# s-esposito/MonoGS

Measured on AMD Instinct MI355X. Metric: rasteriser fwd+bwd Mpix/s @1080p, higher is better.
Workload: dtype f32; 1 GPU; C5: 2000000 Gaussians, 1920x1080, fwd+bwd, seeded synthetic map (SURVEY.md 8d), one keyframe per GPU; gaussians=2000000, width=1920, height=1080, settle_steps=60, instance_count=device-side (capacity mode, overflow checked), parallelism=keyframe-per-gpu x1

## Files before the change

### include/monogs_raster.h

```cpp
#ifndef MONOGS_RASTER_H
#define MONOGS_RASTER_H

#include <stddef.h>
#include <stdint.h>

#ifdef __cplusplus
extern "C" {
#endif

#define MGS_ABI_VERSION 19
#define MGS_TILE 16

typedef struct mgs_camera {
    int32_t image_height;
    int32_t image_width;
    float tanfovx;
    float tanfovy;
    float scale_modifier;
    int32_t sh_degree;
    int32_t sh_coeffs;
    int32_t scale_dim;
    int32_t flags;
    const float* bg;
    const float* viewmatrix;
    const float* projmatrix;
    const float* projmatrix_raw;
    const float* campos;
} mgs_camera;

#define MGS_FLAG_EXCLUSIVE_DEVICE 1

typedef struct mgs_timing {
    float preprocess_ms;
// ... 25 lines not shown
                           const float* opacities,
                           const float* scales,
                           const float* rotations,
                           const float* cov3D_precomp,
                           void* geometry, int32_t* radii ,
                           void* prepare_backward ,
                           uint64_t* num_rendered ,
                           const uint32_t* prev_status ,
                           uint32_t* prev_status_out ,
                           mgs_timing* timing , void* stream);

int mgs_forward_render(const mgs_camera* cam, int32_t P, uint64_t num_rendered,
                       void* geometry, void* binning, void* image,
                       float* out_color, float* out_depth, float* out_opacity, int32_t* n_touched,
                       uint32_t* status ,
                       mgs_timing* timing, void* stream);

#define MGS_STATUS_CAPACITY_OVERFLOW 1u
#define MGS_STATUS_DEPTH_SORT_TIMEOUT 2u
#define MGS_STATUS_TILE_SORT_TIMEOUT 4u

int mgs_debug_set_radix_spin_limit(uint32_t limit);
int mgs_debug_set_option(const char* name, int64_t value);

int mgs_binning_path(int32_t P, int32_t W, int32_t H);

size_t mgs_debug_sort_temp_bytes(uint64_t n, int32_t bits);
int mgs_debug_sort_pairs(uint32_t* keys, uint32_t* vals, uint32_t* keys_alt, uint32_t* vals_alt, uint64_t n, int32_t bits,
                         void* temp, void* stream);

int mgs_forward_render_capacity(const mgs_camera* cam, int32_t P, uint64_t capacity,
                                void* geometry, void* binning, void* image,
                                float* out_color, float* out_depth, float* out_opacity, int32_t* n_touched,
                                uint32_t* overflow, mgs_timing* timing, void* stream);
int mgs_forward_capacity(const mgs_camera* cam, int32_t P, const float* means3D, const float* shs,
                         const float* colors_precomp, const float* opacities, const float* scales, const float* rotations,
                         const float* cov3D_precomp, void* geometry, int32_t* radii, void* prepare_backward,
                         uint64_t capacity, void* binning, void* image, float* out_color, float* out_depth,
                         float* out_opacity, int32_t* n_touched, uint32_t* overflow, mgs_timing* timing, void* stream);

int mgs_backward(const mgs_camera* cam, int32_t P, uint64_t num_rendered,
                 const float* means3D, const float* shs, const float* colors_precomp,
                 const float* opacities, const float* scales, const float* rotations,
                 const float* cov3D_precomp, const int32_t* radii,
                 const void* geometry, const void* binning, const void* image,
                 const float* dL_dcolor, const float* dL_ddepth,
// ... 221 lines not shown
```

### monogs_amd/_lib.py

```python
from __future__ import annotations

import ctypes as C
import os

_HERE = os.path.dirname(os.path.abspath(__file__))
LIB_PATH = os.environ.get("MGS_LIB_PATH") or os.path.join(_HERE, "lib", "libmonogs_raster.so")
ABI_VERSION = 19

c_float_p = C.c_void_p


class MgsCamera(C.Structure):
    _fields_ = [
        ("image_height", C.c_int32), ("image_width", C.c_int32),
        ("tanfovx", C.c_float), ("tanfovy", C.c_float), ("scale_modifier", C.c_float),
        ("sh_degree", C.c_int32), ("sh_coeffs", C.c_int32), ("scale_dim", C.c_int32), ("flags", C.c_int32),
        ("bg", C.c_void_p), ("viewmatrix", C.c_void_p), ("projmatrix", C.c_void_p),
        ("projmatrix_raw", C.c_void_p), ("campos", C.c_void_p),
    ]


class MgsTiming(C.Structure):
    _fields_ = [(n, C.c_float) for n in (
        "preprocess_ms", "depth_sort_ms", "scan_ms", "duplicate_ms", "sort_ms", "ranges_ms", "blend_fwd_ms",
        "blend_bwd_ms", "geom_bwd_ms")]

    def as_dict(self):
        return {n: float(getattr(self, n)) for n, _ in self._fields_}


# ... 33 lines not shown
    "mgs_forward_preprocess": (C.c_int, [C.POINTER(MgsCamera), C.c_int32] + [C.c_void_p] * 7
                               + [C.c_void_p, C.c_void_p, C.c_void_p, C.POINTER(C.c_uint64), C.c_void_p, C.POINTER(C.c_uint32),
                                  C.POINTER(MgsTiming), C.c_void_p]),
    "mgs_forward_capacity": (C.c_int, [C.POINTER(MgsCamera), C.c_int32] + [C.c_void_p] * 7 + [C.c_void_p] * 3 + [C.c_uint64]
                             + [C.c_void_p] * 7 + [C.POINTER(MgsTiming), C.c_void_p]),
    "mgs_forward_render": (C.c_int, [C.POINTER(MgsCamera), C.c_int32, C.c_uint64] + [C.c_void_p] * 8
                           + [C.POINTER(MgsTiming), C.c_void_p]),
    "mgs_debug_set_radix_spin_limit": (C.c_int, [C.c_uint32]),
    "mgs_debug_set_option": (C.c_int, [C.c_char_p, C.c_int64]),
    "mgs_binning_path": (C.c_int, [C.c_int32, C.c_int32, C.c_int32]),
    "mgs_debug_sort_temp_bytes": (C.c_size_t, [C.c_uint64, C.c_int32]),
    "mgs_debug_sort_pairs": (C.c_int, [C.c_void_p] * 4 + [C.c_uint64, C.c_int32, C.c_void_p, C.c_void_p]),
    "mgs_forward_render_capacity": (C.c_int, [C.POINTER(MgsCamera), C.c_int32, C.c_uint64] + [C.c_void_p] * 8
                                    + [C.POINTER(MgsTiming), C.c_void_p]),
    "mgs_backward": (C.c_int, [C.POINTER(MgsCamera), C.c_int32, C.c_uint64] + [C.c_void_p] * 7
                     + [C.c_void_p] * 4 + [C.c_void_p] * 4 + [C.c_void_p] * 9
                     + [C.c_void_p, C.c_int32, C.POINTER(MgsTiming), C.c_void_p]),
    "mgs_backward_tau": (C.c_void_p, [C.c_void_p, C.c_int32]),
    "mgs_debug_blend_stats": (C.c_int, [C.POINTER(MgsCamera), C.c_int32, C.c_uint64] + [C.c_void_p] * 5),
    "mgs_debug_blend_mask_stats": (C.c_int, [C.POINTER(MgsCamera), C.c_int32, C.c_uint64] + [C.c_void_p] * 5),
    "mgs_features_forward": (C.c_int, [C.POINTER(MgsCamera), C.c_int32, C.c_int32, C.c_uint64] + [C.c_void_p] * 7
                             + [C.c_float, C.c_void_p]),
    "mgs_features_backward": (C.c_int, [C.POINTER(MgsCamera), C.c_int32, C.c_int32, C.c_uint64] + [C.c_void_p] * 5 + [C.c_void_p]),
    "mgs_debug_valu_ceiling": (C.c_int, [C.c_void_p, C.c_int32, C.c_void_p]),
    "mgs_debug_set_blend_events": (C.c_int, [C.c_void_p] * 4),
    "mgs_debug_last_backward_split": (C.c_int, []),
    "mgs_mark_visible": (C.c_int, [C.c_int32, C.c_void_p, C.c_void_p, C.c_void_p, C.c_void_p, C.c_void_p]),
    "mgs_loss_scratch_bytes": (C.c_size_t, []),
    "mgs_loss_forward": (C.c_int, [C.c_int32] * 4 + [C.c_float] + [C.c_void_p] * 9 + [C.c_void_p, C.c_void_p, C.c_void_p]),
    "mgs_loss_backward": (C.c_int, [C.c_int32] * 4 + [C.c_float] + [C.c_void_p] * 9
                          + [C.c_void_p, C.c_void_p, C.c_void_p, C.c_void_p, C.c_void_p, C.c_void_p]),
    "mgs_loss_grads": (C.c_int, [C.c_int32] * 4 + [C.c_float] + [C.c_void_p] * 9 + [C.c_void_p] * 4),
    "mgs_ssim_scratch_bytes": (C.c_size_t, [C.c_int32] * 4),
    "mgs_ssim_forward": (C.c_int, [C.c_int32] * 5 + [C.c_float] * 2 + [C.c_void_p] * 5),
    "mgs_ssim_backward": (C.c_int, [C.c_int32] * 4 + [C.c_float] * 2 + [C.c_void_p] * 6),
    "mgs_refine_loss_forward": (C.c_int, [C.c_int32] * 2 + [C.c_float] + [C.c_void_p] * 5),
    "mgs_refine_loss_backward": (C.c_int, [C.c_int32] * 2 + [C.c_float] + [C.c_void_p] * 6),
    "mgs_refine_loss_grads": (C.c_int, [C.c_int32] * 2 + [C.c_float] + [C.c_void_p] * 5),
    "mgs_backproject": (C.c_int, [C.c_int32] * 3 + [C.c_void_p] * 6 + [C.c_float] * 4 + [C.c_void_p] * 6),
    "mgs_camera_setup": (C.c_int, [C.c_void_p] * 7),
    "mgs_pose_step": (C.c_int, [C.c_void_p] * 12 + [C.c_int32] + [C.c_float] * 7
                      + [C.c_void_p, C.c_void_p, C.c_int32, C.c_void_p] + [C.c_void_p] * 4 + [C.c_void_p]),
    "mgs_pose_step_batch": (C.c_int, [C.c_int32, C.POINTER(C.c_void_p)] + [C.c_float] * 7 + [C.c_int32, C.c_void_p]),
    "mgs_adam_step": (C.c_int, [C.c_int32] + [C.c_void_p] * 6 + [C.c_double] * 3 + [C.c_int32, C.c_void_p, C.c_void_p, C.c_void_p]),
    "mgs_window_stats": (C.c_int, [C.c_int32, C.c_int32] + [C.c_void_p] * 6 + [C.c_int32, C.c_void_p, C.c_void_p]),
    "mgs_window_apply": (C.c_int, [C.c_int32] + [C.c_void_p] * 7),
# ... 59 lines not shown
```

### monogs_amd/csrc/api.hip

```cpp
#include "common.h"

#include <stdarg.h>
#include <stdio.h>
#include <string.h>

namespace mgs {

static thread_local char g_err[512] = "";

void set_error(const char* fmt, ...) {
    va_list ap;
    va_start(ap, fmt);
    vsnprintf(g_err, sizeof(g_err), fmt, ap);
    va_end(ap);
}

static inline char* take(char*& p, size_t bytes) {
    char* r = p;
    p += align_up(bytes, 256);
    return r;
}

GeometryState GeometryState::carve(void* base, int P) {
    char* p = (char*)align_up((size_t)base, 256);
// ... 375 lines not shown
    MGS_HIP(zero_fill(stats_dev, MGS_BLEND_STATS_WORDS * sizeof(uint64_t), s));
    if (P == 0 || R == 0) return 0;
    const int W = cam->image_width, H = cam->image_height;
    GeometryState g = GeometryState::carve(const_cast<void*>(geometry), P);
    ImageState img = ImageState::carve(const_cast<void*>(image), W, H);
    BinningState b = BinningState::carve(const_cast<void*>(binning), R, W, H);
    return launch_blend_backward_stats(*cam, g, b, img, (unsigned long long*)stats_dev, s);
}

int mgs_debug_blend_mask_stats(const mgs_camera* cam, int32_t P, uint64_t R, const void* geometry, const void* binning,
                               const void* image, uint64_t* stats_dev, void* stream) {
    if (check_cam(cam)) return 1;
    if (!geometry || !image || !stats_dev || (R > 0 && !binning)) { set_error("bad arguments"); return 1; }
    hipStream_t s = (hipStream_t)stream;
    MGS_HIP(zero_fill(stats_dev, MGS_BLEND_MASK_STATS_WORDS * sizeof(uint64_t), s));
    if (P == 0 || R == 0) return 0;
    const int W = cam->image_width, H = cam->image_height;
    GeometryState g = GeometryState::carve(const_cast<void*>(geometry), P);
    ImageState img = ImageState::carve(const_cast<void*>(image), W, H);
    BinningState b = BinningState::carve(const_cast<void*>(binning), R, W, H);
    return launch_blend_mask_stats(*cam, g, b, img, (unsigned long long*)stats_dev, s);
}

int mgs_debug_valu_ceiling(float* out, int32_t iters, void* stream) {
    if (!out || iters < 1) { set_error("mgs_debug_valu_ceiling: bad arguments"); return 1; }
    return launch_valu_ceiling(out, iters, (hipStream_t)stream);
}

int mgs_debug_last_backward_split(void) { return g_dbg_last_bwd_split; }

int mgs_debug_set_radix_spin_limit(uint32_t limit) { return set_radix_spin_limit(limit); }

int mgs_debug_set_blend_events(void* fwd_start, void* fwd_end, void* bwd_start, void* bwd_end) {
    if ((fwd_start == nullptr) != (fwd_end == nullptr) || (bwd_start == nullptr) != (bwd_end == nullptr)) {
        set_error("mgs_debug_set_blend_events: a pair is both events or neither");
        return 1;
    }
    g_dbg_fwd_events[0] = (hipEvent_t)fwd_start; g_dbg_fwd_events[1] = (hipEvent_t)fwd_end;
    g_dbg_bwd_events[0] = (hipEvent_t)bwd_start; g_dbg_bwd_events[1] = (hipEvent_t)bwd_end;
    return 0;
}

static int g_opt_debug_sort_exclusive = 0;
size_t mgs_debug_sort_temp_bytes(uint64_t n, int32_t bits) { return radix_temp_bytes(n, bits); }
int mgs_debug_sort_pairs(uint32_t* keys, uint32_t* vals, uint32_t* keys_alt, uint32_t* vals_alt, uint64_t n, int32_t bits,
                         void* temp, void* stream) {
// ... 13 lines not shown
    uint32_t err[RADIX_ERROR_WORDS];
    MGS_HIP(hipMemcpyAsync(err, radix_error_flag(temp, n, bits), sizeof(err), hipMemcpyDeviceToHost, s));
    MGS_HIP(hipStreamSynchronize(s));
    if (err[0] | err[1] | err[2] | err[3]) { set_error("mgs_debug_sort_pairs: a look-back spin timed out"); return 2; }
    return 0;
}

int mgs_debug_set_option(const char* name, int64_t value) {
    if (name && !strcmp(name, "radix_scanned")) { g_opt_radix_scanned = (int)value; return 0; }
    if (name && !strcmp(name, "radix_ballot_rank")) { g_opt_radix_ballot_rank = (int)value; return 0; }
    if (name && !strcmp(name, "radix_xcd_band")) { g_opt_radix_xcd_band = (int)value; return 0; }
    if (name && !strcmp(name, "debug_sort_exclusive")) { g_opt_debug_sort_exclusive = (int)value; return 0; }
    if (name && !strcmp(name, "dup_slot_major")) { g_opt_dup_slot_major = (int)value; return 0; }
    if (name && !strcmp(name, "blend_bwd_transposed")) {
        g_opt_blend_bwd_transposed = value < 0 ? 2 : (int)value;
        g_opt_blend_bwd_transposed_set = value >= 0;
        return 0;
    }
    if (name && !strcmp(name, "blend_bwd_split")) { g_opt_blend_bwd_split = value < 0 ? -1 : (int)value; return 0; }
    if (name && !strcmp(name, "blend_bwd_split_min")) { g_opt_blend_bwd_split_min = value < 0 ? 4 : (int)value; return 0; }
    if (name && !strcmp(name, "blend_bwd_split_frac")) { g_opt_blend_bwd_split_frac = value < 0 ? 32 : (int)value; return 0; }
    if (name && !strcmp(name, "scan_small")) { g_opt_scan_small = (int)value; return 0; }
    if (name && !strcmp(name, "tile_sort_fused")) { g_opt_tile_sort_fused = value < 0 ? 1 : (int)value; return 0; }
    if (name && !strcmp(name, "knn_grid_min")) { g_opt_knn_grid_min = value > 0x7FFFFFFF ? 0x7FFFFFFF : (int)value; return 0; }
    set_error("mgs_debug_set_option: unknown option");
    return 1;
}

int mgs_mark_visible(int32_t P, const float* means3D, const float* viewmatrix, const float* projmatrix,
                     uint8_t* visible, void* stream) {
    (void)projmatrix;
    if (P < 0 || (P > 0 && (!means3D || !viewmatrix || !visible))) { set_error("bad arguments"); return 1; }
    return launch_mark_visible(P, means3D, viewmatrix, visible, (hipStream_t)stream);
}

size_t mgs_knn_scratch_bytes(int32_t P) { return knn_scratch_bytes(P); }

int mgs_dist2_knn(int32_t P, const float* points, float* out, void* scratch, void* stream) {
    if (P < 0 || (P > 0 && (!points || !out))) { set_error("bad arguments"); return 1; }
    return launch_knn(P, points, out, scratch, (hipStream_t)stream);
}

}
```

### monogs_amd/csrc/binning.hip

```cpp
#include "common.h"
#include "tile_sort.h"


namespace mgs {

constexpr int SCAN_THREADS = 256;
__device__ __forceinline__ int scan_nblocks_dev(int P) { return (P + SCAN_ITEMS - 1) / SCAN_ITEMS; }
constexpr int SCAN_PER_THREAD = SCAN_ITEMS / SCAN_THREADS;

__device__ __forceinline__ uint32_t wave_incl_scan(uint32_t v, int) { return wave_incl_scan_dpp(v); }

__device__ __forceinline__ uint32_t block_excl_scan(uint32_t v, uint32_t& total, uint32_t* smem ) {
    const int lane = threadIdx.x & 63, wv = threadIdx.x >> 6;
    const uint32_t incl = wave_incl_scan(v, lane);
    if (lane == 63) smem[wv] = incl;
    __syncthreads();
    uint32_t base = 0;
    for (int w = 0; w < wv; ++w) base += smem[w];
    total = smem[0] + smem[1] + smem[2] + smem[3];
    __syncthreads();
    return base + incl - v;
}

__device__ __forceinline__ uint32_t scan_block_rows(const uint2* __restrict__ rects, int n, int cbase, int lane, int wv,
// ... 104 lines not shown
    if (scan_is_small(P)) {
        hipLaunchKernelGGL(scan_small_kernel, dim3(nb), dim3(SCAN_THREADS), 0, s, rects, g.point_offsets, g.scan_blocks,
                           g.scan_status, P, nb, const_cast<uint32_t*>(radix_depth_error_flag(g.sort_temp, (uint64_t)P)),
                           exclusive ? 0 : 1);
        MGS_HIP(hipGetLastError());
        return 0;
    }
    hipLaunchKernelGGL(scan_local_kernel, dim3(nb), dim3(SCAN_THREADS), 0, s, rects, g.point_offsets,
                       g.scan_blocks, P);
    hipLaunchKernelGGL(scan_blocks_kernel, dim3(1), dim3(SCAN_THREADS), 0, s, g.scan_blocks, nb);
    MGS_HIP(hipGetLastError());
    return 0;
}

__device__ __forceinline__ void dup_pair(uint32_t gidx, const uint32_t* __restrict__ depth_key, int lo, uint32_t& val,
                                         uint32_t& kfield) {
    val = gidx; kfield = 0u;
    if (depth_key) {
        const uint32_t k = depth_key[gidx];
        const uint32_t d = k == 0xFFFFFFFFu ? DEPTH_KEY_NARROW : min(k - DEPTH_KEY_SUB, DEPTH_KEY_NARROW);
        kfield = d >> lo;
        if (lo) val |= (d & ((1u << lo) - 1u)) << (32 - lo);
    }
}
__global__ void __launch_bounds__(256) duplicate_kernel(int P, const uint2* __restrict__ rects,
                                                        const uint32_t* __restrict__ perm,
                                                        const uint32_t* __restrict__ depth_key, int tshift, int lo,
                                                        const uint32_t* __restrict__ offsets ,
                                                        const uint32_t* __restrict__ block_sums ,
                                                        uint32_t* keys,
                                                        uint32_t* vals, int gx, int gy, uint32_t r_cap,
                                                        int32_t* __restrict__ n_touched, uint2* __restrict__ ranges,
                                                        int ntiles, uint32_t* __restrict__ zero_ptr, size_t zero_words,
                                                        uint32_t* __restrict__ count, uint32_t* __restrict__ overflow,
                                                        const uint32_t* __restrict__ depth_err, int offsets_global,
                                                        uint32_t* __restrict__ hist , int hist_passes,
                                                        int n_threads , int slot_major,
                                                        unsigned long long* __restrict__ prepare ) {
    const int i = blockIdx.x * 256 + threadIdx.x;
    if (i == 0 && prepare) {
        prepare[1] = prepare[0];
        prepare[0] = 0ull;
    }
    const int lane = threadIdx.x & 63;
    grid_zero(zero_ptr, zero_words, (size_t)n_threads, 256);
    const bool depth_bad = depth_err && radix_failed(depth_err) != 0u;
    if (i == 0 && count) {
        const uint32_t R = (P > 0 && !depth_bad) ? block_sums[scan_nblocks_dev(P)] : 0u;
        count[0] = min(R, r_cap);
        count[1] = R > r_cap ? 1u : 0u;
    }
    if (i == 0 && overflow)
        overflow[0] = (count ? count[1] : 0u) | (depth_bad ? (uint32_t)MGS_STATUS_DEPTH_SORT_TIMEOUT : 0u);
    if (i < ntiles) ranges[i] = make_uint2(0xFFFFFFFFu, 0u);
    if (i < P) n_touched[i] = 0;
    uint32_t idx = 0, nt = 0, off = 0, kf = 0;
    int x0 = 0, y0 = 0, x1 = 0;
    if (i < P) {
        dup_pair(perm ? perm[i] : (uint32_t)i, depth_key, lo, idx, kf);
        const uint2 r = rects[i];
        const int w = (int)(r.y & 0xFFFFu), h = (int)(r.y >> 16);
        nt = (uint32_t)(w * h);
        x0 = (int)(r.x & 0xFFFFu); y0 = (int)(r.x >> 16); x1 = x0 + w;
    }
    if (depth_bad) nt = 0;
    if (nt) off = i == 0 ? 0u : offsets[i - 1] + (offsets_global ? 0u : block_sums[(i - 1) / SCAN_ITEMS]);
    __shared__ uint32_t s_own[4][WAVE];
    __shared__ uint32_t s_idx[4][WAVE], s_off[4][WAVE], s_kf[4][WAVE];
    __shared__ int s_x0[4][WAVE], s_y0[4][WAVE], s_w[4][WAVE];
    __shared__ uint32_t s_hist[2][256];
    if (hist) {
        s_hist[0][threadIdx.x] = 0u; s_hist[1][threadIdx.x] = 0u;
        __syncthreads();
    }
    const int wv = threadIdx.x >> 6;
    if (slot_major) {
        const uint32_t R_all = (P > 0 && !depth_bad) ? block_sums[scan_nblocks_dev(P)] : 0u;
        const uint32_t R_emit = min(R_all, r_cap);
        const uint32_t n_waves = (uint32_t)n_threads / WAVE;
        const uint32_t CH = (((R_emit + n_waves - 1u) / n_waves) + 63u) & ~63u;
        const uint32_t wave_id = (uint32_t)blockIdx.x * 4u + (uint32_t)wv;
        const uint64_t s0w = (uint64_t)wave_id * CH;
        const uint32_t s0 = s0w < (uint64_t)R_emit ? (uint32_t)s0w : R_emit, s1 = (uint64_t)s0 + CH < (uint64_t)R_emit ? s0 + CH : R_emit;
        auto incl = [&](uint32_t k) { return offsets[k] + (offsets_global ? 0u : block_sums[k / SCAN_ITEMS]); };
        uint32_t g = 0;
        if (s0 < s1) {
            uint32_t lo = 0, hi = (uint32_t)P;
            while (hi - lo > 1u) {
                const uint32_t span = hi - lo, step = (span + 63u) / 64u;
                const uint32_t probe = lo + min(((uint32_t)lane + 1u) * step, span) - 1u;
                const unsigned long long above = __builtin_amdgcn_ballot_w64(incl(probe) > s0);
                const int k = __builtin_ctzll(above);
                const uint32_t pk = lo + min(((uint32_t)k + 1u) * step, span) - 1u;
                const uint32_t pk1 = k == 0 ? lo : lo + min((uint32_t)k * step, span);
                lo = pk1; hi = pk + 1u;
            }
            g = lo;
        }
        uint32_t sl = s0;
        while (sl < s1 && g < (uint32_t)P) {
            const uint32_t gi = g + (uint32_t)lane;
            const bool valid = gi < (uint32_t)P;
            uint32_t inc = 0, ntg = 0, idg = 0, kfg = 0;
            int gx0 = 0, gy0 = 0, gw = 1;
            if (valid) {
                inc = incl(gi);
                const uint2 r = rects[gi];
                gw = (int)(r.y & 0xFFFFu);
                ntg = (uint32_t)(gw * (int)(r.y >> 16));
                gx0 = (int)(r.x & 0xFFFFu); gy0 = (int)(r.x >> 16);
                dup_pair(perm ? perm[gi] : gi, depth_key, lo, idg, kfg);
            }
            const uint32_t exc = inc - ntg;
            uint32_t Eg = valid ? inc : 0u;
#pragma unroll
            for (int o2 = 32; o2 > 0; o2 >>= 1) Eg = max(Eg, (uint32_t)__shfl_xor((int)Eg, o2, 64));
            __builtin_amdgcn_wave_barrier();
            s_idx[wv][lane] = idg; s_kf[wv][lane] = kfg; s_off[wv][lane] = exc; s_x0[wv][lane] = gx0; s_y0[wv][lane] = gy0; s_w[wv][lane] = max(gw, 1);
            const uint32_t e = min(s1, Eg);
            const uint32_t cb0 = sl & ~63u;
            const unsigned long long before = __builtin_amdgcn_ballot_w64(ntg != 0u && exc < cb0);
            uint32_t carry = before ? 64u - (uint32_t)__builtin_clzll(before) : 0u;
            for (uint32_t cb = cb0; cb < e; cb += WAVE) {
                __builtin_amdgcn_wave_barrier();
                s_own[wv][lane] = 0u;
                __builtin_amdgcn_wave_barrier();
                if (ntg != 0u && exc >= cb && exc < cb + WAVE) s_own[wv][exc - cb] = (uint32_t)lane + 1u;
                __builtin_amdgcn_wave_barrier();
                uint32_t m = s_own[wv][lane];
#define MGS_DPP_MAX(ctrl, row_mask) m = max(m, (uint32_t)__builtin_amdgcn_update_dpp(0, (int)m, ctrl, row_mask, 0xf, false))
                MGS_DPP_MAX(0x111, 0xf); MGS_DPP_MAX(0x112, 0xf); MGS_DPP_MAX(0x114, 0xf); MGS_DPP_MAX(0x118, 0xf);
                MGS_DPP_MAX(0x142, 0xa); MGS_DPP_MAX(0x143, 0xc);
#undef MGS_DPP_MAX
                const uint32_t owner = max(m, carry);
                carry = (uint32_t)__builtin_amdgcn_readlane((int)owner, 63);
                const uint32_t o = cb + lane;
                if (owner != 0u && o >= sl && o < e) {
                    const uint32_t L = owner - 1u;
                    const uint32_t t = o - s_off[wv][L];
                    const uint32_t w = (uint32_t)s_w[wv][L];
                    const uint32_t yy = t / w, xx = t - yy * w;
                    const uint32_t tid = (uint32_t)((s_y0[wv][L] + (int)yy) * gx + s_x0[wv][L] + (int)xx);
                    const uint32_t key = (tid << tshift) | s_kf[wv][L];
                    keys[o] = key;
                    vals[o] = s_idx[wv][L];
                    if (hist) {
                        atomicAdd(&s_hist[0][(key >> tshift) & 0xFFu], 1u);
                        if (hist_passes > 1) {
                            const uint32_t d1 = (key >> (tshift + 8)) & 0xFFu;
                            const uint32_t lead = (uint32_t)__builtin_amdgcn_readfirstlane((int)d1);
                            const unsigned long long same = __builtin_amdgcn_ballot_w64(d1 == lead);
                            if (d1 != lead) atomicAdd(&s_hist[1][d1], 1u);
                            else if (lane == (int)__builtin_ctzll(same)) atomicAdd(&s_hist[1][lead], (uint32_t)__popcll(same));
                        }
                    }
                }
            }
            sl = max(sl, e);
            if (Eg <= sl) g += WAVE;
        }
        if (hist) {
            __syncthreads();
            const uint32_t c0 = s_hist[0][threadIdx.x], c1 = s_hist[1][threadIdx.x];
            if (c0) atomicAdd(hist + threadIdx.x, c0);
            if (c1) atomicAdd(hist + 256 + threadIdx.x, c1);
        }
        return;
    }
    s_idx[wv][lane] = idx; s_kf[wv][lane] = kf; s_off[wv][lane] = off; s_x0[wv][lane] = x0; s_y0[wv][lane] = y0; s_w[wv][lane] = max(x1 - x0, 1);
    const unsigned long long live = __builtin_amdgcn_ballot_w64(nt != 0);
    if (live == 0ull && !hist) return;
    const int first = live ? __builtin_ctzll(live) : 0, lastl = live ? 63 - __builtin_clzll(live) : 0;
    const uint32_t S = live ? (uint32_t)__builtin_amdgcn_readlane((int)off, first) : 0u;
    const uint32_t E = live ? (uint32_t)__builtin_amdgcn_readlane((int)(off + nt), lastl) : 0u;
    uint32_t carry = 0;
    for (uint32_t cb = S & ~63u; cb < E; cb += WAVE) {
        __builtin_amdgcn_wave_barrier();
        s_own[wv][lane] = 0u;
        __builtin_amdgcn_wave_barrier();
        if (nt != 0 && off >= cb && off < cb + WAVE) s_own[wv][off - cb] = (uint32_t)lane + 1u;
        __builtin_amdgcn_wave_barrier();
        uint32_t m = s_own[wv][lane];
#define MGS_DPP_MAX(ctrl, row_mask) m = max(m, (uint32_t)__builtin_amdgcn_update_dpp(0, (int)m, ctrl, row_mask, 0xf, false))
        MGS_DPP_MAX(0x111, 0xf); MGS_DPP_MAX(0x112, 0xf); MGS_DPP_MAX(0x114, 0xf); MGS_DPP_MAX(0x118, 0xf);
        MGS_DPP_MAX(0x142, 0xa); MGS_DPP_MAX(0x143, 0xc);
#undef MGS_DPP_MAX
        const uint32_t owner = max(m, carry);
        carry = (uint32_t)__builtin_amdgcn_readlane((int)owner, 63);
        const uint32_t o = cb + lane;
        if (owner != 0u && o < E && o < r_cap) {
            const uint32_t L = owner - 1u;
            const uint32_t t = o - s_off[wv][L];
            const uint32_t w = (uint32_t)s_w[wv][L];
            const uint32_t yy = t / w, xx = t - yy * w;
            const uint32_t tid = (uint32_t)((s_y0[wv][L] + (int)yy) * gx + s_x0[wv][L] + (int)xx);
            const uint32_t key = (tid << tshift) | s_kf[wv][L];
            keys[o] = key;
            vals[o] = s_idx[wv][L];
            if (hist) {
                atomicAdd(&s_hist[0][(key >> tshift) & 0xFFu], 1u);
                if (hist_passes > 1) {
                    const uint32_t d1 = (key >> (tshift + 8)) & 0xFFu;
                    const uint32_t lead = (uint32_t)__builtin_amdgcn_readfirstlane((int)d1);
                    const unsigned long long same = __builtin_amdgcn_ballot_w64(d1 == lead);
                    if (d1 != lead) atomicAdd(&s_hist[1][d1], 1u);
                    else if (lane == (int)__builtin_ctzll(same)) atomicAdd(&s_hist[1][lead], (uint32_t)__popcll(same));
                }
            }
        }
    }
    if (hist) {
        __syncthreads();
        const uint32_t c0 = s_hist[0][threadIdx.x], c1 = s_hist[1][threadIdx.x];
        if (c0) atomicAdd(hist + threadIdx.x, c0);
        if (c1) atomicAdd(hist + 256 + threadIdx.x, c1);
    }
}

constexpr uint64_t DUP_SLOT_MAJOR_MIN = 768ull * 1024;
int g_opt_dup_slot_major = -1;

// ... 24 lines not shown
                       zero_words, count, overflow, depth_err,
                       (P > 0 && scan_is_small(P)) ? 1 : 0,
                       count_digits ? g.tile_hist : nullptr, (sort_bits + 7) / 8, n_threads, slot_major ? 1 : 0,
                       P > 0 ? g.prepare : nullptr);
    MGS_HIP(hipGetLastError());
    return 0;
}

size_t sort_temp_bytes(uint64_t n, int bits) { return radix_temp_bytes(n, bits); }

int launch_depth_sort(const GeometryState& g, int P, bool payload, hipStream_t s, bool exclusive) {
    return radix_sort_depth(g.depth_key, g.depth_alt, g.iota, g.iota_alt, g.rect, payload, g.perm, g.rect_sorted, (uint64_t)P,
                            g.sort_temp, s, true, exclusive);
}

int launch_sort(const GeometryState& g, const BinningState& b, uint64_t R, int bits, hipStream_t s, const uint32_t* n_dev,
                bool exclusive, uint2* ranges, bool per_tile) {
    if (R == 0) return 0;
    const bool counted = bits <= 16 && radix_wants_hist(R) && g.tile_hist != nullptr;
    return radix_sort_pairs(b.keys_a, b.vals_a, b.keys_b, b.vals_b, R, bits, b.sort_temp, s, n_dev, true, nullptr, nullptr,
                            counted ? g.tile_hist : nullptr, false, exclusive, ranges, per_tile ? 32 - bits : 0);
}

TileSortArgs tile_sort_args(const mgs_camera& cam, const GeometryState& g, const BinningState& b, uint64_t R,
                            const uint32_t* n_dev) {
    TileSortArgs ts;
    ts.keys = b.keys_sorted;
    ts.vals = b.vals_sorted;
    ts.keys_alt = b.keys_sorted == b.keys_a ? b.keys_b : b.keys_a;
    ts.vals_alt = b.vals_sorted == b.vals_a ? b.vals_b : b.vals_a;
    ts.depth_key = g.depth_key;
    ts.n_dev = n_dev;
    ts.n_cap = (uint32_t)R;
    ts.tb = tile_bits(cam.image_width, cam.image_height);
    return ts;
}

__global__ void __launch_bounds__(TDS_THREADS) tile_depth_sort_kernel(TileSortArgs ts, const uint2* __restrict__ ranges,
                                                                       int ntiles, const uint32_t* __restrict__ sort_err) {
    __shared__ uint32_t s_k[TDS_CAP], s_v[TDS_CAP];
    __shared__ uint32_t s_cnt[TDS_WAVES][TDS_RADIX];
    __shared__ uint32_t s_wsum[TDS_WAVES], s_red[2 * TDS_WAVES];
    const int tile = blockIdx.x;
    if (tile >= ntiles) return;
    tile_depth_sort(ts, ranges[tile], sort_err && radix_failed(sort_err) != 0u, TdsLds{s_k, s_v, s_cnt, s_wsum, s_red});
}

int launch_tile_depth_sort(const mgs_camera& cam, const TileSortArgs& ts, const ImageState& img, const uint32_t* sort_err,
                           hipStream_t s) {
    const int ntiles = tiles_x(cam.image_width) * tiles_y(cam.image_height);
    hipLaunchKernelGGL(tile_depth_sort_kernel, dim3(ntiles), dim3(TDS_THREADS), 0, s, ts, img.ranges, ntiles, sort_err);
    MGS_HIP(hipGetLastError());
    return 0;
}


}
// ... 1 lines not shown
```

### monogs_amd/csrc/common.h

```cpp
#pragma once

#include <hip/hip_runtime.h>
#include <stdint.h>
#include <stddef.h>

#include "../../include/monogs_raster.h"

namespace mgs {

constexpr int TILE = MGS_TILE;
constexpr int WAVE = 64;
constexpr int SUB = 8;
constexpr int REC_FLOATS = 16;
constexpr int GRAD_FLOATS = 16;

enum : int {
    R_X = 0, R_Y = 1, R_EX = 2, R_EY = 3,
    R_CA = 4, R_CB = 5, R_CC = 6, R_OPAC = 7,
    R_R = 8, R_G = 9, R_B = 10, R_DEPTH = 11,
    R_NA = 12, R_NB = 13, R_NC = 14, R_RADIUS = 15
};
enum : int {
    G_SX = 0, G_SY = 1, G_SXX = 2, G_SXY = 3, G_SYY = 4, G_SH = 5,
    G_DR = 6, G_DG = 7, G_DB = 8, G_DDEPTH = 9
// ... 170 lines not shown
                     const uint32_t* ext_hist = nullptr,
                     bool aux_empty_for_ones = false,
                     bool exclusive = false,
                     uint2* ranges = nullptr,
                     int key_shift = 0);
bool radix_wants_hist(uint64_t n);
bool radix_depth_payload(uint64_t n);
int radix_sort_depth(uint32_t* keys, uint32_t* key_b, uint32_t* val_a, uint32_t* val_b, void* rect, bool payload,
                     uint32_t* perm, uint2* rect_sorted, uint64_t n, void* temp, hipStream_t s, bool temp_zeroed,
                     bool exclusive = false);
inline bool depth_sort_payload(int P, int W, int H) { return radix_depth_payload((uint64_t)P) && tiles_x(W) <= 255 && tiles_y(H) <= 255; }
int launch_depth_sort(const GeometryState& g, int P, bool payload, hipStream_t s, bool exclusive = false);
int launch_sort(const GeometryState& g, const BinningState& b, uint64_t R, int bits, hipStream_t s,
                const uint32_t* n_dev = nullptr, bool exclusive = false, uint2* ranges = nullptr, bool per_tile = false);
struct TileSortArgs {
    uint32_t* keys;
    uint32_t* vals;
    uint32_t* keys_alt;
    uint32_t* vals_alt;
    const uint32_t* depth_key;
    const uint32_t* n_dev;
    uint32_t n_cap;
    int tb;
};
TileSortArgs tile_sort_args(const mgs_camera& cam, const GeometryState& g, const BinningState& b, uint64_t R,
                            const uint32_t* n_dev);
int launch_tile_depth_sort(const mgs_camera& cam, const TileSortArgs& ts, const ImageState& img, const uint32_t* sort_err,
                           hipStream_t s);
int set_radix_spin_limit(uint32_t limit);
extern bool g_opt_blend_bwd_transposed_set;
extern int g_dbg_last_bwd_split;
extern int g_opt_radix_ballot_rank, g_opt_radix_scanned, g_opt_radix_xcd_band, g_opt_knn_grid_min, g_opt_scan_small, g_opt_dup_slot_major, g_opt_blend_bwd_transposed, g_opt_blend_bwd_split, g_opt_blend_bwd_split_min, g_opt_blend_bwd_split_frac;
int launch_blend_forward(const mgs_camera& cam, const GeometryState& g, const BinningState& b,
                         const ImageState& img, float* out_color, float* out_depth, float* out_opacity,
                         int32_t* n_touched, const uint32_t* sort_err, uint32_t* status, const TileSortArgs* tile_sort,
                         int P, hipStream_t s);
int launch_blend_backward(const mgs_camera& cam, const GeometryState& g, const BinningState& b,
                          const ImageState& img, const float* dL_dcolor, const float* dL_ddepth, const float* out_color,
                          const float* out_depth, float* grad_acc, bool pose_only, uint64_t num_rendered, hipStream_t s);
int launch_blend_backward_stats(const mgs_camera& cam, const GeometryState& g, const BinningState& b,
                                const ImageState& img, unsigned long long* stats, hipStream_t s);
int launch_blend_mask_stats(const mgs_camera& cam, const GeometryState& g, const BinningState& b,
                            const ImageState& img, unsigned long long* stats, hipStream_t s);
int launch_valu_ceiling(float* out, int iters, hipStream_t s);
int launch_features_forward(const mgs_camera& cam, int P, int K, const GeometryState& g, const BinningState& b,
                            const ImageState& img, const float* features, const float* bg, float* out, int32_t* labels,
                            float min_opacity, hipStream_t s);
int launch_features_backward(const mgs_camera& cam, int P, int K, const GeometryState& g, const BinningState& b,
                             const ImageState& img, const float* dL_dout, float* dL_dfeatures, hipStream_t s);
struct GeomBackwardArgs {
    const float *means3D, *shs, *colors_precomp, *opacities, *scales, *rotations, *cov3D_precomp;
    const int32_t* radii;
    const float* grad_acc;
    float *dL_dmeans2D, *dL_dcolors, *dL_dopacity, *dL_dmeans3D, *dL_dcov3D, *dL_dsh, *dL_dscales,
        *dL_drotations, *dL_dtau;
// ... 11 lines not shown
```

### monogs_amd/csrc/tile_sort.h

```cpp
#pragma once
#include "common.h"

namespace mgs {

constexpr int TDS_THREADS = 256, TDS_WAVES = TDS_THREADS / WAVE, TDS_ITEMS = 4, TDS_CAP = TDS_THREADS * TDS_ITEMS;
constexpr int TDS_DB = 9, TDS_RADIX = 1 << TDS_DB, TDS_DPT = TDS_RADIX / TDS_THREADS;

struct TdsLds {
    uint32_t* k;
    uint32_t* v;
    uint32_t (*cnt)[TDS_RADIX];
    uint32_t* wsum;
    uint32_t* red;
};

__device__ __forceinline__ void tds_minmax(uint32_t lo, uint32_t hi, uint32_t* s_red , uint32_t& mn,
                                           uint32_t& mx) {
    const int lane = threadIdx.x & 63, wv = threadIdx.x >> 6;
#pragma unroll
    for (int o = 32; o > 0; o >>= 1) {
        lo = min(lo, (uint32_t)__shfl_xor((int)lo, o, 64));
        hi = max(hi, (uint32_t)__shfl_xor((int)hi, o, 64));
    }
    if (lane == 0) { s_red[wv] = lo; s_red[TDS_WAVES + wv] = hi; }
    __syncthreads();
    mn = s_red[0]; mx = s_red[TDS_WAVES];
#pragma unroll
    for (int w = 1; w < TDS_WAVES; ++w) { mn = min(mn, s_red[w]); mx = max(mx, s_red[TDS_WAVES + w]); }
    __syncthreads();
}

__device__ __forceinline__ void tds_lds_sort(uint32_t* s_k, uint32_t* s_v, uint32_t (*s_cnt)[TDS_RADIX], uint32_t* s_wsum,
                                             int base, int m, int bits) {
    const int t = threadIdx.x, lane = t & 63, wv = t >> 6;
    for (int sh = 0; sh < bits; sh += TDS_DB) {
#pragma unroll
        for (int w = 0; w < TDS_WAVES; ++w)
#pragma unroll
            for (int j = 0; j < TDS_DPT; ++j) s_cnt[w][t * TDS_DPT + j] = 0u;
        __syncthreads();
        uint32_t k[TDS_ITEMS], v[TDS_ITEMS], r[TDS_ITEMS];
#pragma unroll
        for (int i = 0; i < TDS_ITEMS; ++i) {
            const int e = wv * (TDS_ITEMS * WAVE) + i * WAVE + lane;
            k[i] = 0u; v[i] = 0u; r[i] = 0u;
            if (e < m) {
                k[i] = s_k[base + e]; v[i] = s_v[base + e];
// ... 11 lines not shown
            tsum += tot[j];
        }
        const uint32_t incl = wave_incl_scan_dpp(tsum);
        if (lane == 63) s_wsum[wv] = incl;
        __syncthreads();
        uint32_t run = incl - tsum;
        for (int w = 0; w < wv; ++w) run += s_wsum[w];
#pragma unroll
        for (int j = 0; j < TDS_DPT; ++j)
#pragma unroll
            for (int w = 0; w < TDS_WAVES; ++w) { s_cnt[w][t * TDS_DPT + j] = run; run += c[j][w]; }
        __syncthreads();
#pragma unroll
        for (int i = 0; i < TDS_ITEMS; ++i) {
            const int e = wv * (TDS_ITEMS * WAVE) + i * WAVE + lane;
            if (e < m) {
                const uint32_t dst = s_cnt[wv][(k[i] >> sh) & (TDS_RADIX - 1)] + r[i];
                s_k[base + dst] = k[i]; s_v[base + dst] = v[i];
            }
        }
        __syncthreads();
    }
    __syncthreads();
}

__device__ inline void tds_global_sort(uint32_t* __restrict__ kx, uint32_t* __restrict__ vx, uint32_t* __restrict__ ky,
                                       uint32_t* __restrict__ vy, uint32_t n, const uint32_t* __restrict__ depth_key, int lo,
                                       uint32_t (*s_cnt)[TDS_RADIX], uint32_t* s_run, uint32_t* s_wsum) {
    const int t = threadIdx.x, lane = t & 63, wv = t >> 6;
    const uint32_t imask = lo ? (1u << (32 - lo)) - 1u : 0xFFFFFFFFu;
    for (uint32_t e = t; e < n; e += TDS_THREADS) {
        const uint32_t g = vx[e] & imask;
        kx[e] = depth_key[g] - DEPTH_KEY_SUB;
        vx[e] = g;
    }
    for (int sh = 0; sh < 32; sh += 8) {
        __threadfence();
        if (t < 256) s_run[t] = 0u;
#pragma unroll
        for (int w = 0; w < TDS_WAVES; ++w) s_cnt[w][t] = 0u;
        __syncthreads();
        for (uint32_t e = t; e < n; e += TDS_THREADS) atomicAdd(&s_run[(kx[e] >> sh) & 255u], 1u);
        __syncthreads();
        {
            const uint32_t c = s_run[t], incl = wave_incl_scan_dpp(c);
            if (lane == 63) s_wsum[wv] = incl;
// ... 31 lines not shown
        __threadfence();
        __syncthreads();
        uint32_t* tk = kx; kx = ky; ky = tk;
        uint32_t* tv = vx; vx = vy; vy = tv;
    }
}

__device__ __forceinline__ uint32_t tile_depth_sort(const TileSortArgs& ts, uint2 rg, bool skip, const TdsLds& lds) {
    const int t = threadIdx.x, lane = t & 63, wv = t >> 6;
    const uint32_t n_live = ts.n_dev ? min(ts.n_cap, ts.n_dev[0]) : ts.n_cap;
    const uint32_t start = rg.x, end = min(rg.y, n_live);
    if (skip || start >= end) return 0u;
    const uint32_t n = end - start;
    const int lo = tile_depth_lo_bits(ts.tb);
    const uint32_t kmask = ts.tb < 32 ? (0xFFFFFFFFu >> ts.tb) : 0u, imask = lo ? (1u << (32 - lo)) - 1u : 0xFFFFFFFFu;
    if (n > (uint32_t)TDS_CAP) {
        uint32_t* const k = ts.keys + start;
        uint32_t* const v = ts.vals + start;
        tds_global_sort(k, v, ts.keys_alt + start, ts.vals_alt + start, n, ts.depth_key, lo, lds.cnt, lds.k, lds.wsum);
        return 0u;
    }
    uint32_t d[TDS_ITEMS], g[TDS_ITEMS];
    uint32_t dmin = 0xFFFFFFFFu, dmax = 0u;
#pragma unroll
    for (int i = 0; i < TDS_ITEMS; ++i) {
        const uint32_t e = (uint32_t)(wv * (TDS_ITEMS * WAVE) + i * WAVE + lane);
        d[i] = 0u; g[i] = 0u;
        if (e < n) {
            const uint32_t k = ts.keys[start + e], v = ts.vals[start + e];
            d[i] = ((k & kmask) << lo) | (lo ? v >> (32 - lo) : 0u);
            g[i] = v & imask;
            dmin = min(dmin, d[i]); dmax = max(dmax, d[i]);
        }
    }
    uint32_t mn, mx;
    tds_minmax(dmin, dmax, lds.red, mn, mx);
#pragma unroll
    for (int i = 0; i < TDS_ITEMS; ++i) {
        const int e = wv * (TDS_ITEMS * WAVE) + i * WAVE + lane;
        if (e < (int)n) { lds.k[e] = d[i] - mn; lds.v[e] = g[i]; }
    }
    const uint32_t span = mx - mn;
    tds_lds_sort(lds.k, lds.v, lds.cnt, lds.wsum, 0, (int)n, span ? 32 - __builtin_clz(span) : 0);
    if (mx == DEPTH_KEY_NARROW) {
        uint32_t c = 0;
#pragma unroll
        for (int i = 0; i < TDS_ITEMS; ++i) {
            const uint32_t e = (uint32_t)(wv * (TDS_ITEMS * WAVE) + i * WAVE + lane);
            c += (e < n && d[i] == DEPTH_KEY_NARROW) ? 1u : 0u;
        }
#pragma unroll
        for (int o = 32; o > 0; o >>= 1) c += (uint32_t)__shfl_xor((int)c, o, 64);
        if (lane == 0) lds.red[wv] = c;
        __syncthreads();
        uint32_t m = 0;
#pragma unroll
        for (int w = 0; w < TDS_WAVES; ++w) m += lds.red[w];
        __syncthreads();
        const uint32_t f = n - m;
        uint32_t xmin = 0xFFFFFFFFu, xmax = 0u;
        for (uint32_t e = f + t; e < n; e += TDS_THREADS) {
            const uint32_t x = ts.depth_key[lds.v[e]] - DEPTH_KEY_SUB;
            lds.k[e] = x;
            xmin = min(xmin, x); xmax = max(xmax, x);
        }
        uint32_t rmn, rmx;
// ... 16 lines not shown
```

Measured before the change: 2968 Mpix/s.

## Add bucketed per-tile depth sort, DPP min/max reduction, reciprocal-multiply duplicate slot mapping

The per-tile depth sort gets a bucket path. Keys are scattered into LDS buckets by their top bits, and each key finds its final position by comparing against the other members of its bucket. If any bucket holds more than 32 entries, it falls back to the existing multi-pass LDS radix sort. The min/max reduction now uses DPP row operations instead of shuffles, tile loads are unconditional and clamped, and the duplicate kernel replaces integer division with a precomputed reciprocal and packs per-owner data into vector LDS stores. The bucket path adds extra barriers and an early-exit check, plus a fallback cost on tiles with dense depth clusters.

```diff
diff --git a/include/monogs_raster.h b/include/monogs_raster.h
--- a/include/monogs_raster.h
+++ b/include/monogs_raster.h
@@ -8,7 +8,7 @@
 extern "C" {
 #endif
 
-#define MGS_ABI_VERSION 19
+#define MGS_ABI_VERSION 20
 #define MGS_TILE 16
 
 typedef struct mgs_camera {
@@ -80,6 +80,8 @@
 
 int mgs_debug_set_radix_spin_limit(uint32_t limit);
 int mgs_debug_set_option(const char* name, int64_t value);
+
+int mgs_debug_tile_sort_stats(uint64_t* stats_dev);
 
 int mgs_binning_path(int32_t P, int32_t W, int32_t H);
 
diff --git a/monogs_amd/_lib.py b/monogs_amd/_lib.py
--- a/monogs_amd/_lib.py
+++ b/monogs_amd/_lib.py
@@ -5,7 +5,7 @@
 
 _HERE = os.path.dirname(os.path.abspath(__file__))
 LIB_PATH = os.environ.get("MGS_LIB_PATH") or os.path.join(_HERE, "lib", "libmonogs_raster.so")
-ABI_VERSION = 19
+ABI_VERSION = 20
 
 c_float_p = C.c_void_p
 
@@ -85,6 +85,7 @@
     "mgs_features_forward": (C.c_int, [C.POINTER(MgsCamera), C.c_int32, C.c_int32, C.c_uint64] + [C.c_void_p] * 7
                              + [C.c_float, C.c_void_p]),
     "mgs_features_backward": (C.c_int, [C.POINTER(MgsCamera), C.c_int32, C.c_int32, C.c_uint64] + [C.c_void_p] * 5 + [C.c_void_p]),
+    "mgs_debug_tile_sort_stats": (C.c_int, [C.c_void_p]),
     "mgs_debug_valu_ceiling": (C.c_int, [C.c_void_p, C.c_int32, C.c_void_p]),
     "mgs_debug_set_blend_events": (C.c_int, [C.c_void_p] * 4),
     "mgs_debug_last_backward_split": (C.c_int, []),
diff --git a/monogs_amd/csrc/api.hip b/monogs_amd/csrc/api.hip
--- a/monogs_amd/csrc/api.hip
+++ b/monogs_amd/csrc/api.hip
@@ -421,6 +421,11 @@
     return launch_blend_mask_stats(*cam, g, b, img, (unsigned long long*)stats_dev, s);
 }
 
+int mgs_debug_tile_sort_stats(uint64_t* stats_dev) {
+    g_dbg_tile_sort_stats = (unsigned long long*)stats_dev;
+    return 0;
+}
+
 int mgs_debug_valu_ceiling(float* out, int32_t iters, void* stream) {
     if (!out || iters < 1) { set_error("mgs_debug_valu_ceiling: bad arguments"); return 1; }
     return launch_valu_ceiling(out, iters, (hipStream_t)stream);
@@ -480,6 +485,7 @@
     if (name && !strcmp(name, "blend_bwd_split_frac")) { g_opt_blend_bwd_split_frac = value < 0 ? 32 : (int)value; return 0; }
     if (name && !strcmp(name, "scan_small")) { g_opt_scan_small = (int)value; return 0; }
     if (name && !strcmp(name, "tile_sort_fused")) { g_opt_tile_sort_fused = value < 0 ? 1 : (int)value; return 0; }
+    if (name && !strcmp(name, "tile_sort_bucket")) { g_opt_tile_sort_bucket = value < 0 ? 1 : (int)value; return 0; }
     if (name && !strcmp(name, "knn_grid_min")) { g_opt_knn_grid_min = value > 0x7FFFFFFF ? 0x7FFFFFFF : (int)value; return 0; }
     set_error("mgs_debug_set_option: unknown option");
     return 1;
diff --git a/monogs_amd/csrc/binning.hip b/monogs_amd/csrc/binning.hip
--- a/monogs_amd/csrc/binning.hip
+++ b/monogs_amd/csrc/binning.hip
@@ -150,6 +150,16 @@
         kfield = d >> lo;
         if (lo) val |= (d & ((1u << lo) - 1u)) << (32 - lo);
     }
+}
+__device__ __forceinline__ uint2 dup_owner_div(uint32_t w) {
+    w = max(w, 1u);
+    return make_uint2(w, 0xFFFFFFFFu / w);
+}
+__device__ __forceinline__ uint32_t dup_slot_tile(const uint4 a, const uint2 b, uint32_t o, int gx) {
+    const uint32_t t = o - a.x;
+    uint32_t yy = __umulhi(t, b.y), xx = t - yy * b.x;
+    if (xx >= b.x) { ++yy; xx -= b.x; }
+    return ((a.w >> 16) + yy) * (uint32_t)gx + (a.w & 0xFFFFu) + xx;
 }
 __global__ void __launch_bounds__(256) duplicate_kernel(int P, const uint2* __restrict__ rects,
                                                         const uint32_t* __restrict__ perm,
@@ -182,20 +192,25 @@
         overflow[0] = (count ? count[1] : 0u) | (depth_bad ? (uint32_t)MGS_STATUS_DEPTH_SORT_TIMEOUT : 0u);
     if (i < ntiles) ranges[i] = make_uint2(0xFFFFFFFFu, 0u);
     if (i < P) n_touched[i] = 0;
-    uint32_t idx = 0, nt = 0, off = 0, kf = 0;
-    int x0 = 0, y0 = 0, x1 = 0;
+    uint32_t idx = 0, nt = 0, off = 0, kf = 0, xy = 0, rw = 0;
     if (i < P) {
+        const uint2 r = rects[i];
+        uint32_t o_local = 0, o_block = 0;
+        if (i > 0) {
+            o_local = offsets[i - 1];
+            if (!offsets_global) o_block = block_sums[(i - 1) / SCAN_ITEMS];
+        }
         dup_pair(perm ? perm[i] : (uint32_t)i, depth_key, lo, idx, kf);
-        const uint2 r = rects[i];
-        const int w = (int)(r.y & 0xFFFFu), h = (int)(r.y >> 16);
-        nt = (uint32_t)(w * h);
-        x0 = (int)(r.x & 0xFFFFu); y0 = (int)(r.x >> 16); x1 = x0 + w;
+        off = o_local + o_block;
+        rw = r.y & 0xFFFFu;
+        nt = rw * (r.y >> 16);
+        xy = r.x;
     }
     if (depth_bad) nt = 0;
-    if (nt) off = i == 0 ? 0u : offsets[i - 1] + (offsets_global ? 0u : block_sums[(i - 1) / SCAN_ITEMS]);
+    if (nt == 0) off = 0;
     __shared__ uint32_t s_own[4][WAVE];
-    __shared__ uint32_t s_idx[4][WAVE], s_off[4][WAVE], s_kf[4][WAVE];
-    __shared__ int s_x0[4][WAVE], s_y0[4][WAVE], s_w[4][WAVE];
+    __shared__ uint4 s_oa[4][WAVE];
+    __shared__ uint2 s_ob[4][WAVE];
     __shared__ uint32_t s_hist[2][256];
     if (hist) {
         s_hist[0][threadIdx.x] = 0u; s_hist[1][threadIdx.x] = 0u;
@@ -229,14 +244,13 @@
         while (sl < s1 && g < (uint32_t)P) {
             const uint32_t gi = g + (uint32_t)lane;
             const bool valid = gi < (uint32_t)P;
-            uint32_t inc = 0, ntg = 0, idg = 0, kfg = 0;
-            int gx0 = 0, gy0 = 0, gw = 1;
+            uint32_t inc = 0, ntg = 0, idg = 0, kfg = 0, gxy = 0, gw = 1;
             if (valid) {
                 inc = incl(gi);
                 const uint2 r = rects[gi];
-                gw = (int)(r.y & 0xFFFFu);
-                ntg = (uint32_t)(gw * (int)(r.y >> 16));
-                gx0 = (int)(r.x & 0xFFFFu); gy0 = (int)(r.x >> 16);
+                gw = r.y & 0xFFFFu;
+                ntg = gw * (r.y >> 16);
+                gxy = r.x;
                 dup_pair(perm ? perm[gi] : gi, depth_key, lo, idg, kfg);
             }
             const uint32_t exc = inc - ntg;
@@ -244,7 +258,7 @@
 #pragma unroll
             for (int o2 = 32; o2 > 0; o2 >>= 1) Eg = max(Eg, (uint32_t)__shfl_xor((int)Eg, o2, 64));
             __builtin_amdgcn_wave_barrier();
-            s_idx[wv][lane] = idg; s_kf[wv][lane] = kfg; s_off[wv][lane] = exc; s_x0[wv][lane] = gx0; s_y0[wv][lane] = gy0; s_w[wv][lane] = max(gw, 1);
+            s_oa[wv][lane] = make_uint4(exc, idg, kfg, gxy); s_ob[wv][lane] = dup_owner_div(gw);
             const uint32_t e = min(s1, Eg);
             const uint32_t cb0 = sl & ~63u;
             const unsigned long long before = __builtin_amdgcn_ballot_w64(ntg != 0u && exc < cb0);
@@ -265,13 +279,11 @@
                 const uint32_t o = cb + lane;
                 if (owner != 0u && o >= sl && o < e) {
                     const uint32_t L = owner - 1u;
-                    const uint32_t t = o - s_off[wv][L];
-                    const uint32_t w = (uint32_t)s_w[wv][L];
-                    const uint32_t yy = t / w, xx = t - yy * w;
-                    const uint32_t tid = (uint32_t)((s_y0[wv][L] + (int)yy) * gx + s_x0[wv][L] + (int)xx);
-                    const uint32_t key = (tid << tshift) | s_kf[wv][L];
+                    const uint4 oa = s_oa[wv][L];
+                    const uint32_t tid = dup_slot_tile(oa, s_ob[wv][L], o, gx);
+                    const uint32_t key = (tid << tshift) | oa.z;
                     keys[o] = key;
-                    vals[o] = s_idx[wv][L];
+                    vals[o] = oa.y;
                     if (hist) {
                         atomicAdd(&s_hist[0][(key >> tshift) & 0xFFu], 1u);
                         if (hist_passes > 1) {
@@ -295,7 +307,7 @@
         }
         return;
     }
-    s_idx[wv][lane] = idx; s_kf[wv][lane] = kf; s_off[wv][lane] = off; s_x0[wv][lane] = x0; s_y0[wv][lane] = y0; s_w[wv][lane] = max(x1 - x0, 1);
+    s_oa[wv][lane] = make_uint4(off, idx, kf, xy); s_ob[wv][lane] = dup_owner_div(rw);
     const unsigned long long live = __builtin_amdgcn_ballot_w64(nt != 0);
     if (live == 0ull && !hist) return;
     const int first = live ? __builtin_ctzll(live) : 0, lastl = live ? 63 - __builtin_clzll(live) : 0;
@@ -318,13 +330,11 @@
         const uint32_t o = cb + lane;
         if (owner != 0u && o < E && o < r_cap) {
             const uint32_t L = owner - 1u;
-            const uint32_t t = o - s_off[wv][L];
-            const uint32_t w = (uint32_t)s_w[wv][L];
-            const uint32_t yy = t / w, xx = t - yy * w;
-            const uint32_t tid = (uint32_t)((s_y0[wv][L] + (int)yy) * gx + s_x0[wv][L] + (int)xx);
-            const uint32_t key = (tid << tshift) | s_kf[wv][L];
+            const uint4 oa = s_oa[wv][L];
+            const uint32_t tid = dup_slot_tile(oa, s_ob[wv][L], o, gx);
+            const uint32_t key = (tid << tshift) | oa.z;
             keys[o] = key;
-            vals[o] = s_idx[wv][L];
+            vals[o] = oa.y;
             if (hist) {
                 atomicAdd(&s_hist[0][(key >> tshift) & 0xFFu], 1u);
                 if (hist_passes > 1) {
@@ -395,6 +405,8 @@
                             counted ? g.tile_hist : nullptr, false, exclusive, ranges, per_tile ? 32 - bits : 0);
 }
 
+int g_opt_tile_sort_bucket = 1;
+unsigned long long* g_dbg_tile_sort_stats = nullptr;
 TileSortArgs tile_sort_args(const mgs_camera& cam, const GeometryState& g, const BinningState& b, uint64_t R,
                             const uint32_t* n_dev) {
     TileSortArgs ts;
@@ -406,6 +418,8 @@
     ts.n_dev = n_dev;
     ts.n_cap = (uint32_t)R;
     ts.tb = tile_bits(cam.image_width, cam.image_height);
+    ts.bucket = g_opt_tile_sort_bucket != 0 ? 1 : 0;
+    ts.stats = g_dbg_tile_sort_stats;
     return ts;
 }
 
diff --git a/monogs_amd/csrc/common.h b/monogs_amd/csrc/common.h
--- a/monogs_amd/csrc/common.h
+++ b/monogs_amd/csrc/common.h
@@ -216,15 +216,18 @@
     const uint32_t* n_dev;
     uint32_t n_cap;
     int tb;
+    int bucket;
+    unsigned long long* stats;
 };
 TileSortArgs tile_sort_args(const mgs_camera& cam, const GeometryState& g, const BinningState& b, uint64_t R,
                             const uint32_t* n_dev);
 int launch_tile_depth_sort(const mgs_camera& cam, const TileSortArgs& ts, const ImageState& img, const uint32_t* sort_err,
                            hipStream_t s);
+extern unsigned long long* g_dbg_tile_sort_stats;
 int set_radix_spin_limit(uint32_t limit);
 extern bool g_opt_blend_bwd_transposed_set;
 extern int g_dbg_last_bwd_split;
-extern int g_opt_radix_ballot_rank, g_opt_radix_scanned, g_opt_radix_xcd_band, g_opt_knn_grid_min, g_opt_scan_small, g_opt_dup_slot_major, g_opt_blend_bwd_transposed, g_opt_blend_bwd_split, g_opt_blend_bwd_split_min, g_opt_blend_bwd_split_frac;
+extern int g_opt_radix_ballot_rank, g_opt_radix_scanned, g_opt_radix_xcd_band, g_opt_knn_grid_min, g_opt_scan_small, g_opt_dup_slot_major, g_opt_tile_sort_bucket, g_opt_blend_bwd_transposed, g_opt_blend_bwd_split, g_opt_blend_bwd_split_min, g_opt_blend_bwd_split_frac;
 int launch_blend_forward(const mgs_camera& cam, const GeometryState& g, const BinningState& b,
                          const ImageState& img, float* out_color, float* out_depth, float* out_opacity,
                          int32_t* n_touched, const uint32_t* sort_err, uint32_t* status, const TileSortArgs* tile_sort,
diff --git a/monogs_amd/csrc/tile_sort.h b/monogs_amd/csrc/tile_sort.h
--- a/monogs_amd/csrc/tile_sort.h
+++ b/monogs_amd/csrc/tile_sort.h
@@ -17,12 +17,14 @@
 __device__ __forceinline__ void tds_minmax(uint32_t lo, uint32_t hi, uint32_t* s_red , uint32_t& mn,
                                            uint32_t& mx) {
     const int lane = threadIdx.x & 63, wv = threadIdx.x >> 6;
-#pragma unroll
-    for (int o = 32; o > 0; o >>= 1) {
-        lo = min(lo, (uint32_t)__shfl_xor((int)lo, o, 64));
-        hi = max(hi, (uint32_t)__shfl_xor((int)hi, o, 64));
-    }
-    if (lane == 0) { s_red[wv] = lo; s_red[TDS_WAVES + wv] = hi; }
+    uint32_t nlo = ~lo;
+#define MGS_DPP_MAX2(ctrl, row_mask)                                                                        \
+    nlo = max(nlo, (uint32_t)__builtin_amdgcn_update_dpp(0, (int)nlo, ctrl, row_mask, 0xf, false));          \
+    hi = max(hi, (uint32_t)__builtin_amdgcn_update_dpp(0, (int)hi, ctrl, row_mask, 0xf, false))
+    MGS_DPP_MAX2(0x111, 0xf); MGS_DPP_MAX2(0x112, 0xf); MGS_DPP_MAX2(0x114, 0xf); MGS_DPP_MAX2(0x118, 0xf);
+    MGS_DPP_MAX2(0x142, 0xa); MGS_DPP_MAX2(0x143, 0xc);
+#undef MGS_DPP_MAX2
+    if (lane == 63) { s_red[wv] = ~nlo; s_red[TDS_WAVES + wv] = hi; }
     __syncthreads();
     mn = s_red[0]; mx = s_red[TDS_WAVES];
 #pragma unroll
@@ -80,6 +82,77 @@
         __syncthreads();
     }
     __syncthreads();
+}
+
+constexpr uint32_t TDS_BUCKET_MAX = 32;
+
+__device__ __forceinline__ bool tds_bucket_sort(const TdsLds& lds, const uint32_t (&key)[TDS_ITEMS],
+                                                const uint32_t (&g)[TDS_ITEMS], uint32_t n, int bits) {
+    const int t = threadIdx.x, lane = t & 63, wv = t >> 6;
+    const int sh = bits > TDS_DB ? bits - TDS_DB : 0;
+    uint32_t* const s_tab = &lds.cnt[0][0];
+    uint32_t* const s_bv = &lds.cnt[2][0];
+    static_assert(TDS_WAVES == 4 && 2 * TDS_RADIX == TDS_CAP, "the bucketed indices take the last two counter tables");
+    uint32_t r[TDS_ITEMS];
+#pragma unroll
+    for (int i = 0; i < TDS_ITEMS; ++i) {
+        const uint32_t e = (uint32_t)(wv * (TDS_ITEMS * WAVE) + i * WAVE + lane);
+        r[i] = 0u;
+        if (e < n) r[i] = __hip_atomic_fetch_add(&s_tab[key[i] >> sh], 1u, __ATOMIC_RELAXED, __HIP_MEMORY_SCOPE_WORKGROUP);
+    }
+    __syncthreads();
+    const uint32_t c0 = s_tab[t * TDS_DPT], c1 = s_tab[t * TDS_DPT + 1], tsum = c0 + c1;
+    static_assert(TDS_DPT == 2, "two buckets per thread");
+    if (max(c0, c1) > TDS_BUCKET_MAX) lds.red[0] = 1u;
+    const uint32_t incl = wave_incl_scan_dpp(tsum);
+    if (lane == 63) lds.wsum[wv] = incl;
+    __syncthreads();
+    if (lds.red[0] != 0u) return false;
+    uint32_t run = incl - tsum;
+    for (int w = 0; w < wv; ++w) run += lds.wsum[w];
+    s_tab[t * TDS_DPT] = run | (c0 << 16);
+    s_tab[t * TDS_DPT + 1] = (run + c0) | (c1 << 16);
+    __syncthreads();
+    uint32_t base[TDS_ITEMS], cr[TDS_ITEMS], pos[TDS_ITEMS], cmax = 0u;
+    static_assert(TDS_BUCKET_MAX < 256, "length and slot share a word, a byte each");
+#pragma unroll
+    for (int i = 0; i < TDS_ITEMS; ++i) {
+        const uint32_t e = (uint32_t)(wv * (TDS_ITEMS * WAVE) + i * WAVE + lane);
+        const uint32_t bc = s_tab[e < n ? key[i] >> sh : 0u];
+        base[i] = e < n ? bc & 0xFFFFu : 0u;
+        cr[i] = e < n ? (bc >> 16) | (r[i] << 8) : 0u;
+    }
+#pragma unroll
+    for (int i = 0; i < TDS_ITEMS; ++i) {
+        const uint32_t e = (uint32_t)(wv * (TDS_ITEMS * WAVE) + i * WAVE + lane);
+        if (e < n) { lds.k[base[i] + r[i]] = key[i]; s_bv[base[i] + r[i]] = g[i]; }
+        pos[i] = base[i];
+        cmax = max(cmax, cr[i] & 0xFFu);
+    }
+    __syncthreads();
+    for (uint32_t j = 0; j < cmax; ++j) {
+        uint32_t kk[TDS_ITEMS];
+#pragma unroll
+        for (int i = 0; i < TDS_ITEMS; ++i) kk[i] = lds.k[(base[i] + j) & (uint32_t)(TDS_CAP - 1)];
+        bool any = false;
+#pragma unroll
+        for (int i = 0; i < TDS_ITEMS; ++i) {
+            const bool in = j < (cr[i] & 0xFFu);
+            pos[i] += (in && kk[i] < key[i]) ? 1u : 0u;
+            any = any || (in && kk[i] == key[i] && j != (cr[i] >> 8));
+        }
+        if (__builtin_amdgcn_ballot_w64(any) != 0ull) {
+#pragma unroll
+            for (int i = 0; i < TDS_ITEMS; ++i)
+                if (j < (cr[i] & 0xFFu) && kk[i] == key[i] && j != (cr[i] >> 8) && s_bv[base[i] + j] < g[i]) ++pos[i];
+        }
+    }
+#pragma unroll
+    for (int i = 0; i < TDS_ITEMS; ++i) {
+        const uint32_t e = (uint32_t)(wv * (TDS_ITEMS * WAVE) + i * WAVE + lane);
+        if (e < n) lds.v[pos[i]] = g[i];
+    }
+    return true;
 }
 
 __device__ inline void tds_global_sort(uint32_t* __restrict__ kx, uint32_t* __restrict__ vx, uint32_t* __restrict__ ky,
@@ -157,26 +230,60 @@
     }
     uint32_t d[TDS_ITEMS], g[TDS_ITEMS];
     uint32_t dmin = 0xFFFFFFFFu, dmax = 0u;
-#pragma unroll
-    for (int i = 0; i < TDS_ITEMS; ++i) {
-        const uint32_t e = (uint32_t)(wv * (TDS_ITEMS * WAVE) + i * WAVE + lane);
-        d[i] = 0u; g[i] = 0u;
-        if (e < n) {
-            const uint32_t k = ts.keys[start + e], v = ts.vals[start + e];
-            d[i] = ((k & kmask) << lo) | (lo ? v >> (32 - lo) : 0u);
-            g[i] = v & imask;
-            dmin = min(dmin, d[i]); dmax = max(dmax, d[i]);
-        }
+    {
+        uint32_t kr[TDS_ITEMS], vr[TDS_ITEMS];
+        const uint32_t* const kp = ts.keys + start;
+        const uint32_t* const vp = ts.vals + start;
+#pragma unroll
+        for (int i = 0; i < TDS_ITEMS; ++i) {
+            const uint32_t e = (uint32_t)(wv * (TDS_ITEMS * WAVE) + i * WAVE + lane);
+            const uint32_t at = min(e, n - 1u) & (uint32_t)(TDS_CAP - 1);
+            kr[i] = kp[at]; vr[i] = vp[at];
+        }
+#pragma unroll
+        for (int i = 0; i < TDS_ITEMS; ++i) {
+            const uint32_t e = (uint32_t)(wv * (TDS_ITEMS * WAVE) + i * WAVE + lane);
+            const bool in = e < n;
+            const uint32_t dd = ((kr[i] & kmask) << lo) | (lo ? vr[i] >> (32 - lo) : 0u);
+            d[i] = in ? dd : 0u;
+            g[i] = in ? vr[i] & imask : 0u;
+            dmin = min(dmin, in ? dd : 0xFFFFFFFFu); dmax = max(dmax, d[i]);
+        }
+    }
+    if (ts.bucket) {
+#pragma unroll
+        for (int j = 0; j < TDS_DPT; ++j) lds.cnt[0][t * TDS_DPT + j] = 0u;
     }
     uint32_t mn, mx;
     tds_minmax(dmin, dmax, lds.red, mn, mx);
+    const uint32_t span = mx - mn;
+    const int bits = span ? 32 - __builtin_clz(span) : 0;
+    if (ts.bucket && mx != DEPTH_KEY_NARROW) {
+        if (t == 0) lds.red[0] = 0u;
+        uint32_t key[TDS_ITEMS];
+#pragma unroll
+        for (int i = 0; i < TDS_ITEMS; ++i) key[i] = d[i] - mn;
+        if (tds_bucket_sort(lds, key, g, n, bits)) {
+            if (ts.stats && t == 0) atomicAdd(ts.stats, 1ull);
+            __syncthreads();
+            uint32_t out[TDS_ITEMS];
+#pragma unroll
+            for (int i = 0; i < TDS_ITEMS; ++i) out[i] = lds.v[wv * (TDS_ITEMS * WAVE) + i * WAVE + lane];
+#pragma unroll
+            for (int i = 0; i < TDS_ITEMS; ++i) {
+                const int e = wv * (TDS_ITEMS * WAVE) + i * WAVE + lane;
+                if (e < (int)n) ts.vals[start + e] = out[i];
+            }
+            return n;
+        }
+        if (ts.stats && t == 0) atomicAdd(ts.stats + 1, 1ull);
+    }
 #pragma unroll
     for (int i = 0; i < TDS_ITEMS; ++i) {
         const int e = wv * (TDS_ITEMS * WAVE) + i * WAVE + lane;
         if (e < (int)n) { lds.k[e] = d[i] - mn; lds.v[e] = g[i]; }
     }
-    const uint32_t span = mx - mn;
-    tds_lds_sort(lds.k, lds.v, lds.cnt, lds.wsum, 0, (int)n, span ? 32 - __builtin_clz(span) : 0);
+    tds_lds_sort(lds.k, lds.v, lds.cnt, lds.wsum, 0, (int)n, bits);
     if (mx == DEPTH_KEY_NARROW) {
         uint32_t c = 0;
 #pragma unroll
```

New measurement: 2993 Mpix/s (median of 6 runs). No clear change (+0.8%).
